# andywag/streaming_data_loader

Measured on AMD Instinct MI355X. Metric: device-resident tokenize+mask MB/s of input text, seq_len=512, 1/2/4/8 MI355X, higher is better.
Workload: dtype u8->int32

## Files before the change

streaming_data_loader_amd/csrc/kernels.hpp:

```cpp
#pragma once

#include <hip/hip_runtime.h>

#include <cstdint>

#include "common.hpp"
#include "zstd_format.hpp"

namespace sdl {

hipError_t launch_chunk_ranges(const uint64_t *off, int64_t R, int64_t N, uint32_t *ranges, hipStream_t st,
                               uint32_t *rb1 = nullptr, uint32_t *zero1 = nullptr, const void *copy_src = nullptr,
                               void *copy_dst = nullptr, size_t copy_bytes = 0);

hipError_t launch_wordpiece_chunks(const DevTok &T, const DevFirst &F, bool cased, const uint8_t *text, int64_t N,
                                   const uint64_t *off, int64_t R,
                                   uint32_t *ranges, uint16_t *tokc, uint32_t *chunk_cnt, uint32_t *rec_local,
                                   hipStream_t st, int64_t c_begin = 0, int64_t c_end = -1);

struct BpeLong {
    uint64_t pos;
    uint32_t len;
    uint32_t chunk;
    uint32_t k;
// ... 110 lines not shown
                             uint64_t n_order, uint8_t *windows, uint16_t *gmaps, uint8_t *gwin, hipStream_t st);
hipError_t launch_gz_resolve(const uint16_t *slots, uint32_t cap, const uint32_t *order, const uint32_t *len,
                             const uint64_t *pos, uint64_t n_order, const uint8_t *windows, uint8_t *out,
                             uint32_t *crc, uint32_t *shift, const X2N &x2n, int32_t *status, hipStream_t st);
hipError_t launch_gz_crc_fold(const uint32_t *crc, const uint32_t *shift, uint64_t n_order, const uint8_t *trailer,
                              const int32_t *status, int32_t *mstatus, hipStream_t st);

int64_t scan_tmp_words(int64_t n);
hipError_t launch_exclusive_scan(const uint32_t *in, uint32_t *out, int64_t n, uint32_t *tmp, hipStream_t st,
                                 const uint32_t *carry_in = nullptr);
int64_t scan_small_max();

enum : int32_t {
    ZS_OK = zs::OK,
    ZS_E_RANGE = zs::E_RANGE,
    ZS_E_TRUNC = zs::E_TRUNC,
    ZS_E_MAGIC = zs::E_MAGIC,
    ZS_E_DICT = zs::E_DICT,
    ZS_E_WINDOW = zs::E_WINDOW,
    ZS_E_BTYPE = zs::E_BTYPE,
    ZS_E_BSIZE = zs::E_BSIZE,
    ZS_E_LITHDR = zs::E_LITHDR,
    ZS_E_HUF = zs::E_HUF,
    ZS_E_FSE = zs::E_FSE,
    ZS_E_SEQHDR = zs::E_SEQHDR,
    ZS_E_ENDBITS = zs::E_ENDBITS,
    ZS_E_FAR = zs::E_FAR,
    ZS_E_SIZE = zs::E_SIZE,
    ZS_E_CHECKSUM = zs::E_CHECKSUM,
    ZS_E_STALL = zs::E_STALL
};
hipError_t launch_zs_index(const uint8_t *zst, uint64_t len, const uint64_t *foff, uint64_t n, zs::Frame *frames,
                           zs::Block *blocks, const uint32_t *first_block, uint32_t *nblk, uint32_t block_cap,
                           hipStream_t st);
hipError_t launch_zs_parse(const uint8_t *zst, const zs::Frame *frames, zs::Block *blocks, uint32_t nb, hipStream_t st);
hipError_t launch_zs_link(zs::Frame *frames, zs::Block *blocks, uint64_t n, uint32_t *lit_tot, uint32_t *seq_tot,
                          unsigned long long *totals, hipStream_t st);
hipError_t launch_zs_decode(const uint8_t *zst, const zs::Frame *frames, zs::Block *blocks, uint32_t nb,
                            const uint32_t *lit_base, const uint32_t *seq_base, uint8_t *lit, zs::SeqRec *seq,
                            hipStream_t st);
hipError_t launch_zs_chain(zs::Frame *frames, zs::Block *blocks, uint64_t n, uint32_t *out_size,
                           unsigned long long *totals, hipStream_t st);
hipError_t launch_zs_write(const uint8_t *zst, zs::Frame *frames, const zs::Block *blocks, uint32_t nb, uint64_t n,
                           const uint32_t *lit_base, const uint32_t *seq_base, const uint8_t *lit, const zs::SeqRec *seq,
                           const uint32_t *ooff, uint8_t *out, bool check, int32_t *status, uint32_t *bad,
                           hipStream_t st, hipEvent_t *ev = nullptr);

constexpr int MAX_SEGMENTS = 16;
struct SegChunks {
    int64_t cb[MAX_SEGMENTS + 1];
    int K;
};
hipError_t launch_seg_bounds(const uint32_t *ranges, const SegChunks &sc, int64_t R, uint32_t *rb, hipStream_t st);
hipError_t launch_scan_range(const uint32_t *in, uint32_t *out, const uint32_t *rb, int k, hipStream_t st);

hipError_t launch_compact_tokens(const uint32_t *tokc, const uint32_t *chunk_cnt, const uint32_t *chunk_off,
                                 int64_t n_chunks, uint32_t *tok, const uint32_t *long_count,
                                 const uint32_t *chunk_ent, const BpeLong *long_list, const uint16_t *long_scratch,
                                 hipStream_t st, const uint32_t *long_pool = nullptr, int64_t stride = STAGE,
                                 bool list16 = false);


struct SegSel {
    const uint32_t *rb;
    int k;
    int last;
};

int64_t records_tile_words(int64_t R);
hipError_t launch_records(const RowParams &P, const uint64_t *off, int64_t R, int64_t N, const uint32_t *chunk_off,
                          int64_t n_chunks, const uint32_t *rec_local, uint32_t *rec_tok, uint32_t *rec_cnt,
                          uint32_t *rec_rows, SegSel sel, hipStream_t st, uint32_t *tile_sums = nullptr);

struct DirectDst {
    int32_t *ids[2], *am[2], *tt[2], *lab[2];
    uint32_t base, cap, B, pad;
};
struct RowOut {
    int32_t *input_ids, *attention_mask, *token_type_ids, *labels;
    float *labels_f32;
    DirectDst direct;
};

constexpr int64_t SMALL_CHUNKS = 64;
struct SmallDown {
    const uint32_t *tokc, *chunk_cnt;
    uint32_t *chunk_off, *tok;
    const uint32_t *long_count, *chunk_ent;
    const BpeLong *long_list;
    const uint16_t *long_scratch;
    const uint32_t *long_pool;
    int64_t stride;
    int list16;
    const uint32_t *rec_local;
    uint32_t *rec_tok, *rec_cnt, *rec_rows, *row_off, *row_rec;
    uint32_t *stat;
    const uint32_t *tok_err;
    int rows;
    RowOut out;
};
hipError_t launch_downstream_small(const SmallDown &d, const RowParams &P, const uint64_t *off, int64_t R, int64_t N,
                                   hipStream_t st);

struct TokSrc {
    const uint32_t *tok;
    const uint16_t *lists;
    const uint32_t *chunk_off;
    int64_t n_lists;
    const uint32_t *row_chunk;
};

struct RowChunkIn {
    uint32_t *row_chunk;
    const uint32_t *rec_tok, *rec_cnt, *chunk_off;
    const uint64_t *off;
    int64_t n_lists;
    int32_t S, n_pre, chunk;
};
hipError_t launch_row_map(const uint32_t *row_off, int64_t R, uint32_t *row_rec, SegSel sel, hipStream_t st,
                          const RowChunkIn *rc = nullptr);
hipError_t launch_scan_rows_map(const uint32_t *rec_rows, int64_t R, const uint32_t *tile_sums, uint32_t *row_off,
                                uint32_t *row_rec, hipStream_t st, const RowChunkIn *rc = nullptr);

struct RowSeg {
    int32_t *ids, *am, *tt, *lab;
    uint32_t g0, n, dst, pad;
};
hipError_t launch_rows_to_host(const RowSeg *segs, int n_segs, uint32_t rows_per_seg_max, const int32_t *ids,
                               const int32_t *am, const int32_t *tt, const int32_t *lab, int S, int LW,
                               hipStream_t st);

hipError_t launch_rows_direct(const DirectDst &d, const uint32_t *row_off, int64_t R, const int32_t *ids,
                              const int32_t *am, const int32_t *tt, const int32_t *lab, int S, int LW,
                              const uint32_t *err0, const uint32_t *err1, uint32_t *stat, hipStream_t st);

struct MaskPolicy {
    int32_t policy;
    int32_t per_mille;
    uint32_t vocab_size;
    uint32_t pad;
    const uint32_t *cont_bits;
};

hipError_t launch_rows(const RowParams &P, const TokSrc &src, const uint32_t *rec_tok, const uint32_t *rec_cnt,
                       const uint32_t *row_off, const uint32_t *row_rec, SegSel sel, int64_t rows_cap, RowOut out,
                       hipStream_t st,
                       hipStream_t st_late = nullptr, const MaskPolicy *mp = nullptr);
struct PackParams {
    const uint32_t *tok, *rec_tok, *rec_cnt;
    uint32_t *rec_len;
    uint32_t *pk_off;
    int64_t R, rows_cap;
    int32_t S, B, eos, min_ids;
    const int32_t *carry_ids, *carry_pos;
    const uint32_t *carry_len;
    int32_t *new_ids, *new_pos;
    uint32_t *new_len;
    int32_t *ids, *am, *lab, *pos;
    uint32_t *d_rows;
};
hipError_t launch_pack_lengths(const PackParams &q, hipStream_t st);
hipError_t launch_pack_rows(const PackParams &q, hipStream_t st);
hipError_t launch_pack_flush(const PackParams &q, hipStream_t st);

struct PairParams {
    const uint16_t *lists;
    const uint32_t *chunk_off;
    const uint64_t *off;
    int64_t n_lists;
    const uint32_t *rec_tok, *rec_cnt;
    int64_t n_pairs;
    int64_t rows_end;
    int32_t S, cls, sep, pad;
    int32_t *ids, *am, *tt;
    uint32_t *row_off, *row_rec, *rb;
};
hipError_t launch_rows_pair(const PairParams &q, hipStream_t st);

hipError_t launch_mask_rand_rec(const RowParams &P, uint32_t *list, uint32_t *spos, uint16_t *jbuf, uint32_t *bits,
                                hipStream_t st);
hipError_t launch_multi_labels(const uint32_t *labels, const uint64_t *label_off, const uint32_t *row_rec,
                               const uint32_t *row_off, SegSel sel, int64_t rows_cap, int B, int NL, float *out,
                               uint32_t *err, hipStream_t st);

struct SpanPlan {
    uint2 *tab;
    uint2 *meta;
    int32_t capr;
    uint32_t *ovf_list, *ovf_n;
};
hipError_t launch_rows_span(const RowParams &P, const uint32_t *tok, const uint32_t *rec_tok, const uint32_t *rec_cnt,
                            const uint32_t *row_off, const uint32_t *row_rec, SegSel sel, int64_t rows_cap,
                            RowOut out, uint32_t *err, hipStream_t st, const SpanPlan *plan = nullptr);

// ... 41 lines not shown
```

streaming_data_loader_amd/csrc/pipeline.hip:

```cpp
#include "common.hpp"
#include "device_util.hpp"
#include "kernels.hpp"
#include "rows_device.hpp"
#include "span_noise.hpp"

namespace sdl {

constexpr int SCAN_NT = 256;
constexpr int SCAN_PER = 8;
constexpr int SCAN_TILE = SCAN_NT * SCAN_PER;
constexpr int64_t SCAN_MAX_BLOCKS = 1024;

__global__ __launch_bounds__(SCAN_NT) void k_scan_reduce(const uint32_t *__restrict__ in, int64_t n,
                                                         uint32_t *__restrict__ sums, int64_t nb,
                                                         const uint32_t *carry_in) {
    __shared__ uint32_t scratch[SCAN_NT / 64];
    const int64_t base = (int64_t)blockIdx.x * SCAN_TILE + (int64_t)threadIdx.x * SCAN_PER;
    uint32_t s = 0;
#pragma unroll
    for (int k = 0; k < SCAN_PER; ++k)
        if (base + k < n) s += in[base + k];
    uint32_t tot;
    block_excl_sum<SCAN_NT>(s, &tot, scratch);
    if (threadIdx.x == 0) {
// ... 478 lines not shown
    ChaRow cr;
    chacha_row_init(cr, key);
    uint32_t *gnx = nx + (S + 1) * grp, *gbt = bt + bw * grp;
    for (int x = gl; x <= S; x += 16) gnx[x] = NONE;
    for (int x = gl; x < bw; x += 16) gbt[x] = 0u;
    int i = active ? S - 1 : 0;
    uint32_t n = (uint32_t)i + 1u, zone = (n << __builtin_clz(n)) - 1u;
    for (uint32_t blk = 0;; blk += 16) {
        const int irow = __builtin_amdgcn_update_dpp(0, i, 0x150, 0xF, 0xF, false);
        if (!__any(irow >= i0)) break;
        uint32_t o[16];
        chacha12_block_row(cr, blk + (uint32_t)gl, o);
        static_for<0, 16>([&](auto bc) {
            constexpr int b = decltype(bc)::value;
#pragma unroll
            for (int q = 0; q < 16; ++q) {
                const uint32_t x = (uint32_t)__builtin_amdgcn_update_dpp(0, (int)o[q], 0x150 + b, 0xF, 0xF, false);
                const uint64_t m = (uint64_t)x * n;
                const bool acc = i >= i0 && (uint32_t)m <= zone;
                const uint32_t j = (uint32_t)(m >> 32);
                if (gl == 0) atomicMin(&gnx[acc && j != (uint32_t)i ? j : (uint32_t)S], (uint32_t)i);
                i -= acc ? 1 : 0;
                n = (uint32_t)i + 1u;
                zone = (n << __builtin_clz(n)) - 1u;
            }
        });
    }
    wave_sync();
    if (active)
        for (int x = gl; x < kmask; x += 16) {
            uint32_t p = (uint32_t)x;
            for (uint32_t q = gnx[p]; q != NONE; q = gnx[p]) p = q;
            atomicOr(&gbt[p >> 5], 1u << (p & 31));
        }
    wave_sync();
}

template <int MR, bool RM1, bool LATE = false, bool LISTS = false>
__global__ __launch_bounds__(256) __attribute__((amdgpu_waves_per_eu(MR >= 4 ? ROWS_WAVES4 : LATE ? 4 : RM1 ? ROWS_WAVES_RM1 : ROWS_WAVES, 8))) void k_rows(RowParams P, TokSrc tok,
                                              const uint32_t *__restrict__ rec_tok, const uint32_t *__restrict__ rec_cnt,
                                              const uint32_t *__restrict__ row_off, const uint32_t *__restrict__ row_rec,
                                              SegSel sel, int64_t rows_cap, RowOut out) {
    const int lane = lane_id();
    const int wid = LISTS ? __builtin_amdgcn_readfirstlane((int)(threadIdx.x >> 6)) : (int)(threadIdx.x >> 6);
    constexpr int NXS = 256 * MR + 1, BW = 8 * MR;
    __shared__ __attribute__((aligned(16))) uint32_t s_rw[LATE ? 4 : 1][LATE ? 4 * (NXS + BW) : 1];
    const RowSpan rs = row_span(sel, row_off, P.B, rows_cap);
    const int64_t G = rs.g_real;
    const DirectDst &dd = out.direct;
    const int64_t g_end = dd.cap ? rs.g_real : rs.g_end;
    if constexpr (LATE) {
        for (int64_t g0 = rs.g_lo + ((int64_t)blockIdx.x * 4 + wid) * 64; g0 < G; g0 += (int64_t)gridDim.x * 256) {
            const int64_t gl = g0 + lane;
            bool late = false;
            if (gl < G) {
                const int64_t r = row_rec[gl];
                late = rand_pre_slot(P, r, (uint32_t)(gl - row_off[r])) < 0;
            }
            uint32_t *const rw = s_rw[LATE ? wid : 0];
            uint32_t *const bits = rw + 4 * NXS;
            for (uint64_t m = __ballot(late); m;) {
                const int nr = __popcll(m) < 4 ? __popcll(m) : 4;
                uint64_t mm = m;
                for (int q = 0; q < (lane >> 4) && mm; ++q) mm &= mm - 1;
                const int64_t gq = g0 + (mm ? __builtin_ctzll(mm) : 0);
                uint64_t rec = 0;
                uint32_t kq = 0;
                if ((lane >> 4) < nr) {
                    const int64_t r = row_rec[gq];
                    rec = P.first_record + (uint64_t)r;
                    kq = (uint32_t)(gq - row_off[r]);
                }
                rand_rows16(P, nr, rec, kq, rw, bits, BW, lane);
                for (int q = 0; q < nr; ++q, m &= m - 1)
                    row_one<MR, RM1, LATE, LISTS>(P, tok, rec_tok, rec_cnt, row_off, row_rec, g0 + __builtin_ctzll(m), G, out,
                                           bits + BW * q, lane);
                __builtin_amdgcn_wave_barrier();
            }
        }
    } else {
        for (int64_t g = rs.g_lo + (int64_t)blockIdx.x * 4 + wid; g < g_end; g += (int64_t)gridDim.x * 4)
            row_one<MR, RM1, LATE, LISTS>(P, tok, rec_tok, rec_cnt, row_off, row_rec, g, G, out, nullptr, lane);
    }
}

template <int MR, bool WHOLE, bool LISTS>
__global__ __launch_bounds__(256) void k_rows_policy(RowParams P, MaskPolicy mp, TokSrc tok,
                                                     const uint32_t *__restrict__ rec_tok,
                                                     const uint32_t *__restrict__ rec_cnt,
                                                     const uint32_t *__restrict__ row_off,
                                                     const uint32_t *__restrict__ row_rec, SegSel sel,
                                                     int64_t rows_cap, RowOut out) {
    const int lane = lane_id();
    const int wid = __builtin_amdgcn_readfirstlane((int)(threadIdx.x >> 6));
    __shared__ uint32_t s_unit[WHOLE ? 4 : 1][WHOLE ? 256 * MR : 1];
    const RowSpan rs = row_span(sel, row_off, P.B, rows_cap);
    const int64_t G = rs.g_real;
    const int64_t g_end = out.direct.cap ? rs.g_real : rs.g_end;
    for (int64_t g = rs.g_lo + (int64_t)blockIdx.x * 4 + wid; g < g_end; g += (int64_t)gridDim.x * 4)
        row_policy_one<MR, WHOLE, LISTS>(P, mp, tok, rec_tok, rec_cnt, row_off, row_rec, g, G, out,
                                         s_unit[WHOLE ? wid : 0], lane);
}

template <int MR>
__global__ __launch_bounds__(SCAN_SMALL_NT) void k_downstream_small(SmallDown d, RowParams P,
                                                                    const uint64_t *__restrict__ off, int64_t R,
                                                                    int64_t N, int64_t n_chunks) {
    __shared__ uint32_t scratch[SCAN_SMALL_NT / 64];
    block_scan_small(d.chunk_cnt, n_chunks, d.chunk_off, scratch);
    __syncthreads();
    for (int64_t cb = (int64_t)(threadIdx.x >> 6) * COMPACT_CPW; cb < n_chunks;
         cb += (int64_t)(SCAN_SMALL_NT / 64) * COMPACT_CPW)
        compact_small(d, cb, d.chunk_off, n_chunks);
    for (int64_t r = threadIdx.x; r < R; r += SCAN_SMALL_NT)
        record_one(P, off, r, N, d.chunk_off, n_chunks, d.rec_local, d.rec_tok, d.rec_cnt, d.rec_rows);
    __syncthreads();
    block_scan_small(d.rec_rows, R, d.row_off, scratch);
    __syncthreads();
    for (int64_t r = threadIdx.x; r < R; r += SCAN_SMALL_NT)
        for (uint32_t g = d.row_off[r]; g < d.row_off[r + 1]; ++g) d.row_rec[g] = (uint32_t)r;
    if (d.stat) {
        for (int64_t r = threadIdx.x; r <= R; r += SCAN_SMALL_NT) d.stat[r] = d.row_off[r];
        if (threadIdx.x == 0) {
            d.stat[R + 1] = 0u;
            d.stat[R + 2] = d.tok_err ? *d.tok_err : 0u;
        }
    }
    if constexpr (MR > 0) {
        __syncthreads();
        const int64_t G = (int64_t)d.row_off[R];
        const int64_t g_end = d.out.direct.cap ? G : (G + P.B - 1) / P.B * P.B;
        for (int64_t g = (int64_t)(threadIdx.x >> 6); g < g_end; g += SCAN_SMALL_NT / 64)
            row_one<MR, false, false>(P, TokSrc{d.tok}, d.rec_tok, d.rec_cnt, d.row_off, d.row_rec, g, G, d.out, nullptr,
                                      lane_id());
    }
}

template <int MR>
__global__ __launch_bounds__(64) void k_downstream_tiny(SmallDown d, RowParams P, const uint64_t *__restrict__ off,
                                                        int64_t R, int64_t N, int64_t n_chunks) {
    downstream_tiny<MR>(d, P, off, R, N, n_chunks);
}

hipError_t launch_downstream_small(const SmallDown &d, const RowParams &P, const uint64_t *off, int64_t R, int64_t N,
                                   hipStream_t st) {
    const int64_t n_chunks = (N + CHUNK - 1) / CHUNK;
    if (n_chunks > SMALL_CHUNKS || R > SCAN_SMALL) return hipErrorInvalidValue;
    const int MR = (P.S + 255) / 256;
    if (d.rows && ((P.rng_mode == 1 && P.task == 0) || (P.task != 0 && P.task != 1)))
        return hipErrorInvalidValue;
    const bool tiny = R <= 64 && n_chunks <= 64;
#define LAUNCH_DS(M)                                                                                                    \
    if (tiny) hipLaunchKernelGGL(k_downstream_tiny<M>, dim3(1), dim3(64), 0, st, d, P, off, R, N, n_chunks);        \
    else hipLaunchKernelGGL(k_downstream_small<M>, dim3(1), dim3(SCAN_SMALL_NT), 0, st, d, P, off, R, N, n_chunks)
    if (!d.rows) LAUNCH_DS(0);
    else if (MR <= 1) LAUNCH_DS(1);
    else if (MR <= 2) LAUNCH_DS(2);
    else if (MR <= 4) LAUNCH_DS(4);
    else if (MR <= 8) LAUNCH_DS(8);
    else return hipErrorInvalidValue;
#undef LAUNCH_DS
    return hipGetLastError();
}

template <int NR>
__device__ __forceinline__ void rand_walk_lanes(const RowParams &P, const bool (&active)[NR], const uint64_t (&rec)[NR],
// ... 237 lines not shown
                                                     int S, int LW, const uint32_t *__restrict__ err0,
                                                     const uint32_t *__restrict__ err1, uint32_t *__restrict__ stat) {
    if (blockIdx.x == 0) {
        for (int64_t r = threadIdx.x; r <= R; r += 256) stat[r] = row_off[r];
        if (threadIdx.x == 0) {
            stat[R + 1] = err0 ? *err0 : 0u;
            stat[R + 2] = err1 ? *err1 : 0u;
        }
    }
    const uint32_t total = row_off[R];
    const uint32_t n = total < d.cap ? total : d.cap;
    const int plane = (int)(threadIdx.x >> 6), lane = (int)(threadIdx.x & 63);
    const int32_t *src = plane == 0 ? ids : plane == 1 ? am : plane == 2 ? tt : lab;
    if (!src) return;
    const int W = plane == 3 ? LW : S;
    const bool vec = (W & 3) == 0;
    for (uint32_t g = blockIdx.x; g < n; g += gridDim.x) {
        const uint32_t slot = d.base + g, bi = slot >= d.B ? 1u : 0u, row = slot - bi * d.B;
        int32_t *dst = plane == 0 ? d.ids[bi] : plane == 1 ? d.am[bi] : plane == 2 ? d.tt[bi] : d.lab[bi];
        const int32_t *s = src + (size_t)g * W;
        int32_t *o = dst + (size_t)row * W;
        if (vec && ((uintptr_t)dst & 15u) == 0) {
            for (int j = 4 * lane; j < W; j += 256)
                *reinterpret_cast<int4 *>(o + j) = *reinterpret_cast<const int4 *>(s + j);
        } else {
            for (int j = lane; j < W; j += 64) o[j] = s[j];
        }
    }
}

hipError_t launch_rows_direct(const DirectDst &d, const uint32_t *row_off, int64_t R, const int32_t *ids,
                              const int32_t *am, const int32_t *tt, const int32_t *lab, int S, int LW,
                              const uint32_t *err0, const uint32_t *err1, uint32_t *stat, hipStream_t st) {
    const unsigned grid = d.cap < 64u ? (d.cap ? d.cap : 1u) : 64u;
    hipLaunchKernelGGL(k_rows_direct, dim3(grid), dim3(256), 0, st, d, row_off, R, ids, am, tt, lab, S, LW, err0, err1,
                       stat);
    return hipGetLastError();
}

hipError_t launch_rows(const RowParams &P, const TokSrc &tok, const uint32_t *rec_tok, const uint32_t *rec_cnt,
                       const uint32_t *row_off, const uint32_t *row_rec, SegSel sel, int64_t rows_cap, RowOut out,
                       hipStream_t st, hipStream_t st_late, const MaskPolicy *mp) {
    if (!st_late) st_late = st;
    if (rows_cap == 0) return hipSuccess;
    if (mp && mp->policy != 0) {
        if (P.task != 0 || P.rng_mode != 0 || mp->policy < 1 || mp->policy > 2 || P.label_width != P.S ||
            !out.labels || (mp->policy == 2 && !mp->cont_bits))
            return hipErrorInvalidValue;
        const int64_t want_p = (rows_cap + 3) / 4;
        const unsigned grid_p = (unsigned)(want_p < 16384 ? want_p : 16384);
        const int MRp = (P.S + 255) / 256;
#define LAUNCH_POLICY_L(MM, WW, LL)                                                                                     \
    hipLaunchKernelGGL((k_rows_policy<MM, WW, LL>), dim3(grid_p), dim3(256), 0, st, P, *mp, tok, rec_tok, rec_cnt,   \
                       row_off, row_rec, sel, rows_cap, out)
#define LAUNCH_POLICY(MM)                                                                                               \
    do {                                                                                                              \
        if (mp->policy == 2) {                                                                                        \
            if (tok.lists) LAUNCH_POLICY_L(MM, true, true);                                                           \
            else LAUNCH_POLICY_L(MM, true, false);                                                                    \
        } else {                                                                                                      \
            if (tok.lists) LAUNCH_POLICY_L(MM, false, true);                                                          \
            else LAUNCH_POLICY_L(MM, false, false);                                                                   \
        }                                                                                                             \
    } while (0)
        if (MRp <= 1) LAUNCH_POLICY(1);
        else if (MRp <= 2) LAUNCH_POLICY(2);
        else if (MRp <= 4) LAUNCH_POLICY(4);
        else if (MRp <= 8) LAUNCH_POLICY(8);
        else return hipErrorInvalidValue;
#undef LAUNCH_POLICY
#undef LAUNCH_POLICY_L
        return hipGetLastError();
    }
constexpr int ROWS_GRID_CAP = 16384;
    const int64_t want = (rows_cap + 3) / 4;
    const unsigned grid = (unsigned)(want < ROWS_GRID_CAP ? want : ROWS_GRID_CAP);
    const int MR = (P.S + 255) / 256;
    if (P.label_width > 256 * MR) return hipErrorInvalidValue;
    const bool rm1 = P.task == 0 && P.rng_mode == 1;
    if (rm1 && ((P.mask_bits0 && !P.mask_off) || P.mask_w * 32 < P.S || P.S > RAND_MAX_S))
        return hipErrorInvalidValue;
    const int64_t want_late = (rows_cap + 255) / 256;
    const unsigned grid_late = (unsigned)(want_late < 2048 ? want_late : 2048);
#define LAUNCH_ROWS_L(MM, LL)                                                                                           \
    if (rm1) {                                                                                                        \
        hipLaunchKernelGGL((k_rows<MM, true, false, LL>), dim3(grid), dim3(256), 0, st, P, tok, rec_tok, rec_cnt,    \
                           row_off, row_rec, sel, rows_cap, out);                                                     \
        hipLaunchKernelGGL((k_rows<MM, true, true, LL>), dim3(grid_late), dim3(256), 0, st_late, P, tok, rec_tok,    \
                           rec_cnt, row_off, row_rec, sel, rows_cap, out);                                            \
    } else                                                                                                            \
        hipLaunchKernelGGL((k_rows<MM, false, false, LL>), dim3(grid), dim3(256), 0, st, P, tok, rec_tok, rec_cnt,   \
                           row_off, row_rec, sel, rows_cap, out)
#define LAUNCH_ROWS(MM)                                                                                                 \
    do {                                                                                                              \
        if (tok.lists) {                                                                                              \
            LAUNCH_ROWS_L(MM, true);                                                                                  \
        } else {                                                                                                      \
            LAUNCH_ROWS_L(MM, false);                                                                                 \
        }                                                                                                             \
    } while (0)
    if (MR <= 1) LAUNCH_ROWS(1);
    else if (MR <= 2) LAUNCH_ROWS(2);
    else if (MR <= 4) LAUNCH_ROWS(4);
    else if (MR <= 8) LAUNCH_ROWS(8);
    else return hipErrorInvalidValue;
#undef LAUNCH_ROWS
#undef LAUNCH_ROWS_L
    return hipGetLastError();
}

__device__ __forceinline__ uint32_t span_pick(int32_t kmin, int32_t n, const uint32_t (&thr)[32], uint32_t x) {
    int32_t v = kmin;
#pragma unroll
    for (int j = 0; j < 32; ++j) v += (j < n && thr[j] <= x) ? 1 : 0;
    return (uint32_t)v;
}

constexpr int SPAN_WBLK = 17;
constexpr int SPAN_WU64 = 8 * SPAN_WBLK;
constexpr double ZIG_R = 3.6541528853610088;

struct SpanStream {
    uint32_t key[8];
    const uint32_t *win;
    uint64_t wblk;
    uint32_t cblk[16];
    int64_t chave;
    __device__ uint64_t at(uint64_t k) {
        const uint64_t b = k >> 3;
        uint32_t lo, hi;
        if (b - wblk < (uint64_t)SPAN_WBLK) {
            const uint32_t w = (uint32_t)(2 * (k - 8 * wblk));
            lo = win[w];
            hi = win[w + 1];
        } else {
            if ((int64_t)b != chave) {
                chacha12_block(key, (uint32_t)b, cblk);
                chave = (int64_t)b;
            }
            lo = cblk[2 * (k & 7)];
            hi = cblk[2 * (k & 7) + 1];
        }
        return (uint64_t)hi << 32 | lo;
    }
};

__device__ __forceinline__ double bits_f64(uint64_t b) { return __longlong_as_double((long long)b); }

__device__ __forceinline__ bool zig_fast(uint64_t bits, const double *__restrict__ ZX, double *x) {
#pragma clang fp contract(off)
    const int i = (int)(bits & 0xffu);
    const double u = bits_f64((bits >> 12) | (1024ull << 52)) - 3.0;
    *x = u * ZX[i];
    return fabs(*x) < ZX[i + 1];
}

template <class Stream>
__device__ double zig_normal(Stream &s, uint64_t k, const double *__restrict__ ZX,
                             const double *__restrict__ ZF, uint32_t *len) {
#pragma clang fp contract(off)
    const uint64_t k0 = k;
    for (;;) {
        const uint64_t bits = s.at(k++);
        const int i = (int)(bits & 0xffu);
        const double u = bits_f64((bits >> 12) | (1024ull << 52)) - 3.0;
        const double x = u * ZX[i];
// ... 868 lines not shown
```

streaming_data_loader_amd/csrc/rows_device.hpp:

```cpp
#pragma once
#include "common.hpp"
#include "device_util.hpp"
#include "kernels.hpp"
#include "list_index.hpp"
#include "mlm_pick.hpp"

namespace sdl {

static_assert(LIST_CHUNK == CHUNK && LIST_STRIDE == STAGE, "list_index.hpp restates the chunk geometry");

constexpr int COMPACT_CPW = 4;
template <int PART = 0, bool E16 = false>
__device__ __forceinline__ void compact_wave(int64_t cb, const uint32_t *__restrict__ tokc,
                                             const uint32_t *__restrict__ chunk_cnt,
                                             const uint32_t *__restrict__ chunk_off, int64_t n_chunks,
                                             uint32_t *__restrict__ tok, const uint32_t *long_count,
                                             const uint32_t *__restrict__ chunk_ent,
                                             const BpeLong *__restrict__ long_list,
                                             const uint16_t *__restrict__ long_scratch,
                                             const uint32_t *__restrict__ long_pool, int64_t stride) {
    const int lane = threadIdx.x & 63;
    uint32_t n[COMPACT_CPW], o[COMPACT_CPW];
#pragma unroll
    for (int j = 0; j < COMPACT_CPW; ++j) {
// ... 404 lines not shown
            mwd[m] = j0 < S && mine ? bw[j0 >> 5] : 0u;
        }
        if (LATE) __builtin_amdgcn_wave_barrier();
    }

    const RowIds<MR> ids = row_ids<MR, LISTS>(P, src, c, bnd, nl, t0, cnt, base, l, lane);
    const int32_t (&id)[MR][4] = ids.v;
    if (RM1 && !mine) return;
    const int tail0 = l < S ? S - l : S;
    const uint64_t rec = P.first_record + (uint64_t)r;
    if (P.task == 0) {
        bool sel[MR][4];
        if (RM1) {
#pragma unroll
            for (int m = 0; m < MR; ++m) {
                const int j0 = 256 * m + 4 * lane;
#pragma unroll
                for (int w = 0; w < 4; ++w) sel[m][w] = (mwd[m] >> ((j0 + w) & 31)) & 1u;
            }
        } else {
            uint32_t key[MR][4];
#pragma unroll
            for (int m = 0; m < MR; ++m) {
                const uint4 c = philox4x32_10(make_uint4((uint32_t)(64 * m + lane), k, (uint32_t)rec,
                                                         (uint32_t)(rec >> 32)),
                                              (uint32_t)P.seed, (uint32_t)(P.seed >> 32));
                const int j0 = 256 * m + 4 * lane;
                key[m][0] = j0 < S ? c.x : 0xFFFFFFFFu;
                key[m][1] = j0 + 1 < S ? c.y : 0xFFFFFFFFu;
                key[m][2] = j0 + 2 < S ? c.z : 0xFFFFFFFFu;
                key[m][3] = j0 + 3 < S ? c.w : 0xFFFFFFFFu;
            }
            select_k_smallest_interp<MR>(key, P.mask_length, S < 256 * MR ? S : 256 * MR, sel);
        }
#pragma unroll
        for (int m = 0; m < MR; ++m) {
            const int j0 = 256 * m + 4 * lane;
            int32_t v[4], lab[4], am[4];
#pragma unroll
            for (int w = 0; w < 4; ++w) {
                v[w] = id[m][w];
                lab[w] = -100;
                if (sel[m][w] && v[w] != 0) {
                    lab[w] = v[w];
                    v[w] = P.mask_id;
                }
                am[w] = j0 + w >= tail0 ? 0 : 1;
            }
            store4(ids_o, j0, S, vec, v[0], v[1], v[2], v[3]);
            store4(am_o, j0, S, vec, am[0], am[1], am[2], am[3]);
            if (tt_o) store4(tt_o, j0, S, vec, 0, 0, 0, 0);
            store4(lb_o, j0, P.label_width, vec_lb, lab[0], lab[1], lab[2], lab[3]);
        }
    } else if (P.task == 3 || P.task == 4) {
#pragma unroll
        for (int m = 0; m < MR; ++m) {
            const int j0 = 256 * m + 4 * lane;
            int32_t am[4];
#pragma unroll
            for (int w = 0; w < 4; ++w) am[w] = j0 + w >= tail0 ? 0 : 1;
            store4(ids_o, j0, S, vec, id[m][0], id[m][1], id[m][2], id[m][3]);
            store4(am_o, j0, S, vec, am[0], am[1], am[2], am[3]);
            if (tt_o) store4(tt_o, j0, S, vec, 0, 0, 0, 0);
        }
    } else {
#pragma unroll
        for (int m = 0; m < MR; ++m) {
            const int j0 = 256 * m + 4 * lane;
            int32_t am[4], lab[4];
#pragma unroll
            for (int w = 0; w < 4; ++w) {
                const bool tail = j0 + w >= tail0;
                am[w] = tail ? 0 : 1;
                lab[w] = tail ? -100 : id[m][w];
            }
            store4(ids_o, j0, S, vec, id[m][0], id[m][1], id[m][2], id[m][3]);
            store4(am_o, j0, S, vec, am[0], am[1], am[2], am[3]);
            if (tt_o) store4(tt_o, j0, S, vec, 0, 0, 0, 0);
            store4(lb_o, j0, P.label_width, vec_lb, lab[0], lab[1], lab[2], lab[3]);
        }
    }
}

__device__ __forceinline__ uint32_t max_u32(uint32_t a, uint32_t b) { return a > b ? a : b; }
__device__ __forceinline__ uint32_t min_u32r(uint32_t a, uint32_t b) { return a < b ? a : b; }
struct PickWave {
    uint32_t l;
    __device__ __forceinline__ uint32_t sum(uint32_t x) const {
        return (uint32_t)__builtin_amdgcn_readlane((int)wave_incl_sum(x), 63);
    }
    __device__ __forceinline__ uint32_t min(uint32_t x) const {
        DPP_SCAN_ID(x, min_u32r, 0xFFFFFFFFu);
        return (uint32_t)__builtin_amdgcn_readlane((int)x, 63);
    }
    __device__ __forceinline__ uint32_t lane() const { return l; }
};

template <int MR, bool WHOLE, bool LISTS>
__device__ __forceinline__ void row_policy_one(const RowParams &P, const MaskPolicy &mp, const TokSrc &src,
                                               const uint32_t *__restrict__ rec_tok,
                                               const uint32_t *__restrict__ rec_cnt,
                                               const uint32_t *__restrict__ row_off,
                                               const uint32_t *__restrict__ row_rec, int64_t g, int64_t G,
                                               const RowOut &out, uint32_t *lds, int lane) {
    const int S = P.S;
    const bool vec = (S & 3) == 0;
    const DirectDst &dd = out.direct;
    int32_t *ids_o = out.input_ids + g * S;
    int32_t *am_o = out.attention_mask + g * S;
    int32_t *tt_o = out.token_type_ids ? out.token_type_ids + g * S : nullptr;
    int32_t *lb_o = out.labels + g * (int64_t)S;
    if (g < (int64_t)dd.cap) {
        const uint32_t slot = dd.base + (uint32_t)g, bi = slot >= dd.B ? 1u : 0u, row = slot - bi * dd.B;
        ids_o = dd.ids[bi] + (size_t)row * S;
        am_o = dd.am[bi] + (size_t)row * S;
        tt_o = dd.tt[bi] ? dd.tt[bi] + (size_t)row * S : nullptr;
        lb_o = dd.lab[bi] + (size_t)row * S;
    }
    if (g >= (int64_t)G) {
#pragma unroll
        for (int m = 0; m < MR; ++m) {
            const int j0 = 256 * m + 4 * lane;
            store4(ids_o, j0, S, vec, 0, 0, 0, 0);
            store4(am_o, j0, S, vec, 1, 1, 1, 1);
            if (tt_o) store4(tt_o, j0, S, vec, 0, 0, 0, 0);
            store4(lb_o, j0, S, vec, -100, -100, -100, -100);
        }
        return;
    }
    const int64_t nl = LISTS ? src.n_lists : 0;
    uint32_t c = 0, bnd = 0;
    if constexpr (LISTS) {
        c = (uint32_t)__builtin_amdgcn_readfirstlane((int)src.row_chunk[g]);
        bnd = src.chunk_off[(int64_t)c + lane < nl ? (int64_t)c + lane : nl];
    }
    const int64_t r = row_rec[g];
    const uint32_t ck = (uint32_t)(g - row_off[r]);
    const uint32_t cnt = rec_cnt[r];
    const uint32_t t0 = rec_tok[r];
    const int64_t n = (int64_t)cnt + P.n_pre + P.n_post;
    const int64_t base = P.chunk ? (int64_t)ck * S : 0;
    const int l = (int)((n - base) < S ? (n - base) : S);
    const RowIds<MR> ids = row_ids<MR, LISTS>(P, src, c, bnd, nl, t0, cnt, base, l, lane);
    const int32_t (&id)[MR][4] = ids.v;
    const int tail0 = l < S ? S - l : S;
    const uint64_t rec = P.first_record + (uint64_t)r;
    const PickWave wv{(uint32_t)lane};

    uint32_t cand = 0;
#pragma unroll
    for (int m = 0; m < MR; ++m)
#pragma unroll
        for (int w = 0; w < 4; ++w) {
            const int32_t v = id[m][w];
            bool ex = v == 0 || v == P.mask_id;
#pragma unroll
            for (int q = 0; q < MAX_FRAME; ++q)
                ex = ex || (q < P.n_pre && v == frame_id(P.pre, q)) || (q < P.n_post && v == frame_id(P.post, q));
            if (256 * m + 4 * lane + w < l && !ex) cand |= 1u << (4 * m + w);
        }
    const int ncand = (int)wv.sum((uint32_t)__popc(cand));
    int kb = (int)(((int64_t)l * mp.per_mille + 500) / 1000);
    kb = kb < 1 ? 1 : kb;
    kb = kb < P.mask_length ? kb : P.mask_length;
    if (ncand == 0) kb = 0;

// ... 183 lines not shown
```

Baseline: 241,500.

## Add specialized fast row-building kernel reading args from kernarg segment

Adds a k_rows_fast kernel, specialised per task, for the common row-building configuration: aligned S, no direct destinations, default RNG mode. It reads parameters straight from the kernarg segment with scalar-pinned reloads to keep register pressure down, sets waves-per-EU occupancy hints, and writes output with vectorised nontemporal stores. The aim is to cut VGPR/SGPR pressure and branching in the generic row kernel, at the cost of a second code path that has to stay semantically in sync with the original (padding rows, frames, MLM selection).

```diff
diff --git a/streaming_data_loader_amd/csrc/kernels.hpp b/streaming_data_loader_amd/csrc/kernels.hpp
--- a/streaming_data_loader_amd/csrc/kernels.hpp
+++ b/streaming_data_loader_amd/csrc/kernels.hpp
@@ -216,6 +216,13 @@
     DirectDst direct;
 };
 
+struct RowFast {
+    int32_t *input_ids, *attention_mask, *token_type_ids, *labels;
+    uint64_t seed, first_record;
+    int32_t S, B, chunk, mask_length, mask_id, n_pre, n_post, pad;
+    int32_t pre[MAX_FRAME], post[MAX_FRAME];
+};
+
 constexpr int64_t SMALL_CHUNKS = 64;
 struct SmallDown {
     const uint32_t *tokc, *chunk_cnt;
@@ -244,6 +251,15 @@
     const uint32_t *row_chunk;
 };
 
+struct RowsFastArgs {
+    RowFast F;
+    TokSrc tok;
+    const uint32_t *rec_tok, *rec_cnt, *row_off, *row_rec;
+    const uint32_t *rb;
+    int32_t k, last;
+    int64_t rows_cap;
+};
+
 struct RowChunkIn {
     uint32_t *row_chunk;
     const uint32_t *rec_tok, *rec_cnt, *chunk_off;
diff --git a/streaming_data_loader_amd/csrc/pipeline.hip b/streaming_data_loader_amd/csrc/pipeline.hip
--- a/streaming_data_loader_amd/csrc/pipeline.hip
+++ b/streaming_data_loader_amd/csrc/pipeline.hip
@@ -584,6 +584,24 @@
         for (int64_t g = rs.g_lo + (int64_t)blockIdx.x * 4 + wid; g < g_end; g += (int64_t)gridDim.x * 4)
             row_one<MR, RM1, LATE, LISTS>(P, tok, rec_tok, rec_cnt, row_off, row_rec, g, G, out, nullptr, lane);
     }
+}
+
+template <int MR, int TASK, bool LISTS>
+__global__ __launch_bounds__(256) __attribute__((amdgpu_waves_per_eu(MR >= 4 ? ROWS_WAVES4 : ROWS_WAVES, 8))) void k_rows_fast(
+    RowsFastArgs A) {
+    const int lane = lane_id();
+    const uint32_t wid = (uint32_t)__builtin_amdgcn_readfirstlane((int)(threadIdx.x >> 6));
+    const uint32_t g_lo = A.row_off[A.rb[A.k]], G = A.row_off[A.rb[A.k + 1]], step = gridDim.x * 4u;
+    uint32_t g_end = G;
+    if (A.last) {
+        const uint32_t B = (uint32_t)A.F.B, cap = (uint32_t)A.rows_cap;
+        uint32_t pad = (G + B - 1u) / B * B;
+        pad = pad > cap ? cap : pad;
+        g_end = pad > G ? pad : G;
+    }
+    const RowArgs a = (RowArgs)__builtin_amdgcn_kernarg_segment_ptr();
+    for (uint32_t g = g_lo + blockIdx.x * 4u + wid; g < g_end; g += step)
+        row_fast_one<MR, TASK, LISTS>(a, g, G, lane);
 }
 
 template <int MR, bool WHOLE, bool LISTS>
@@ -987,6 +1005,41 @@
         return hipErrorInvalidValue;
     const int64_t want_late = (rows_cap + 255) / 256;
     const unsigned grid_late = (unsigned)(want_late < 2048 ? want_late : 2048);
+    const bool label_task = P.task == 3 || P.task == 4;
+    const bool fast = (P.S & 3) == 0 && out.direct.cap == 0 && P.rng_mode == 0 && rows_cap < (int64_t(1) << 31) &&
+                      (label_task || ((P.task == 0 || P.task == 1) && out.labels && P.label_width == P.S));
+    if (fast) {
+        RowsFastArgs A{RowFast{out.input_ids, out.attention_mask, out.token_type_ids, label_task ? nullptr : out.labels,
+                               P.seed, P.first_record, P.S, P.B, P.chunk, P.mask_length, P.mask_id, P.n_pre, P.n_post,
+                               0, {}, {}},
+                       tok, rec_tok, rec_cnt, row_off, row_rec, sel.rb, sel.k, sel.last, rows_cap};
+        for (int q = 0; q < MAX_FRAME; ++q) {
+            A.F.pre[q] = P.pre[q];
+            A.F.post[q] = P.post[q];
+        }
+#define LAUNCH_FAST_L(MM, TT, LL)                                                                                       \
+    hipLaunchKernelGGL((k_rows_fast<MM, TT, LL>), dim3(grid), dim3(256), 0, st, A)
+#define LAUNCH_FAST(MM)                                                                                                 \
+    do {                                                                                                              \
+        if (tok.lists) {                                                                                              \
+            if (label_task) LAUNCH_FAST_L(MM, ROW_LABELS, true);                                                      \
+            else if (P.task == 0) LAUNCH_FAST_L(MM, ROW_MLM, true);                                                   \
+            else LAUNCH_FAST_L(MM, ROW_CLM, true);                                                                    \
+        } else {                                                                                                      \
+            if (label_task) LAUNCH_FAST_L(MM, ROW_LABELS, false);                                                     \
+            else if (P.task == 0) LAUNCH_FAST_L(MM, ROW_MLM, false);                                                  \
+            else LAUNCH_FAST_L(MM, ROW_CLM, false);                                                                   \
+        }                                                                                                             \
+    } while (0)
+        if (MR <= 1) LAUNCH_FAST(1);
+        else if (MR <= 2) LAUNCH_FAST(2);
+        else if (MR <= 4) LAUNCH_FAST(4);
+        else if (MR <= 8) LAUNCH_FAST(8);
+        else return hipErrorInvalidValue;
+#undef LAUNCH_FAST
+#undef LAUNCH_FAST_L
+        return hipGetLastError();
+    }
 #define LAUNCH_ROWS_L(MM, LL)                                                                                           \
     if (rm1) {                                                                                                        \
         hipLaunchKernelGGL((k_rows<MM, true, false, LL>), dim3(grid), dim3(256), 0, st, P, tok, rec_tok, rec_cnt,    \
diff --git a/streaming_data_loader_amd/csrc/rows_device.hpp b/streaming_data_loader_amd/csrc/rows_device.hpp
--- a/streaming_data_loader_amd/csrc/rows_device.hpp
+++ b/streaming_data_loader_amd/csrc/rows_device.hpp
@@ -510,6 +510,235 @@
     }
 }
 
+constexpr int ROW_MLM = 0, ROW_CLM = 1, ROW_LABELS = 2;
+
+typedef const __attribute__((address_space(4))) RowsFastArgs *RowArgs;
+__device__ __forceinline__ RowArgs row_args_again(RowArgs a) {
+    asm volatile("" : "+s"(a));
+    return a;
+}
+
+__device__ __forceinline__ void store4v(int32_t *p, int j0, int32_t a, int32_t b, int32_t c, int32_t d) {
+    typedef int32_t v4i __attribute__((ext_vector_type(4)));
+    __builtin_nontemporal_store(v4i{a, b, c, d}, reinterpret_cast<v4i *>(p + j0));
+}
+
+template <int MR, bool LISTS>
+__device__ __forceinline__ RowIds<MR> row_ids_fast(RowArgs a, uint32_t c, uint32_t bnd, int64_t nl, uint32_t t0,
+                                                   uint32_t cnt, int64_t base, int l, int lane) {
+    const int n_pre = a->F.n_pre;
+    const int64_t rel0 = base > n_pre ? base - n_pre : 0;
+    const int64_t rel1 = base + l - n_pre < (int64_t)cnt ? base + l - n_pre : (int64_t)cnt;
+    const int jlo = (int)(rel0 + n_pre - base), jhi = (int)(rel1 + n_pre - base);
+    const uint32_t tb = t0 + (uint32_t)(base - n_pre);
+    RowIds<MR> out;
+#pragma unroll
+    for (int m = 0; m < MR; ++m)
+#pragma unroll
+        for (int w = 0; w < 4; ++w) out.v[m][w] = 0;
+    if (rel0 < rel1) {
+        uint32_t t[MR][4];
+#pragma unroll
+        for (int m = 0; m < MR; ++m)
+#pragma unroll
+            for (int w = 0; w < 4; ++w) {
+                const int j = 256 * m + 4 * lane + w;
+                const int jc = j < jlo ? jlo : j > jhi - 1 ? jhi - 1 : j;
+                t[m][w] = tb + (uint32_t)jc;
+            }
+        if constexpr (LISTS) {
+            const uint32_t t_last = (uint32_t)__builtin_amdgcn_readfirstlane((int)(tb + (uint32_t)(jhi - 1)));
+            const uint16_t *__restrict__ lc = a->tok.lists + (int64_t)c * STAGE;
+            if ((uint32_t)__builtin_amdgcn_readlane((int)bnd, 63) > t_last) {
+                uint32_t q[MR][4];
+#pragma unroll
+                for (int m = 0; m < MR; ++m)
+#pragma unroll
+                    for (int w = 0; w < 4; ++w) q[m][w] = 0;
+#pragma unroll 1
+                for (int b = 1; b < 64; ++b) {
+                    const uint32_t x = (uint32_t)__builtin_amdgcn_readlane((int)bnd, b);
+                    if (x > t_last) break;
+#pragma unroll
+                    for (int m = 0; m < MR; ++m)
+#pragma unroll
+                        for (int w = 0; w < 4; ++w) q[m][w] += t[m][w] >= x ? 1u : 0u;
+                }
+#pragma unroll
+                for (int m = 0; m < MR; ++m)
+#pragma unroll
+                    for (int w = 0; w < 4; ++w) {
+                        const uint32_t lo = (uint32_t)__shfl((int)bnd, (int)(q[m][w] & 63u));
+                        out.v[m][w] = (int32_t)lc[q[m][w] * (uint32_t)STAGE + (t[m][w] - lo)];
+                    }
+            } else {
+                const uint32_t *const chunk_off = a->tok.chunk_off;
+                const uint16_t *const lists = a->tok.lists;
+#pragma unroll 1
+                for (int i = 0; i < 4 * MR; ++i) {
+                    uint32_t ti = 0;
+#pragma unroll
+                    for (int m = 0; m < MR; ++m)
+#pragma unroll
+                        for (int w = 0; w < 4; ++w) ti = i == 4 * m + w ? t[m][w] : ti;
+                    const int64_t cc = list_chunk_of(chunk_off, (int64_t)c, nl - 1, ti);
+                    const int32_t v = (int32_t)lists[list_slot(chunk_off, cc, ti)];
+#pragma unroll
+                    for (int m = 0; m < MR; ++m)
+#pragma unroll
+                        for (int w = 0; w < 4; ++w) out.v[m][w] = i == 4 * m + w ? v : out.v[m][w];
+                }
+            }
+        } else {
+            const uint32_t *const tok = a->tok.tok;
+#pragma unroll
+            for (int m = 0; m < MR; ++m)
+#pragma unroll
+                for (int w = 0; w < 4; ++w) out.v[m][w] = (int32_t)tok[t[m][w]];
+        }
+    }
+    a = row_args_again(a);
+    static_assert(MAX_FRAME == 4, "the frame selects below");
+    int32_t p0 = a->F.pre[0], p1 = a->F.pre[1], p2 = a->F.pre[2], p3 = a->F.pre[3];
+    int32_t q0 = a->F.post[0], q1 = a->F.post[1], q2 = a->F.post[2], q3 = a->F.post[3];
+    asm volatile("" : "+s"(p0), "+s"(p1), "+s"(p2), "+s"(p3), "+s"(q0), "+s"(q1), "+s"(q2), "+s"(q3));
+    auto frame4 = [](int k, int32_t x0, int32_t x1, int32_t x2, int32_t x3) {
+        int32_t x = x3;
+        x = k == 2 ? x2 : x;
+        x = k == 1 ? x1 : x;
+        x = k == 0 ? x0 : x;
+        return x;
+    };
+    const int post0 = (int)(base - n_pre - (int64_t)cnt);
+#pragma unroll
+    for (int m = 0; m < MR; ++m)
+#pragma unroll
+        for (int w = 0; w < 4; ++w) {
+            const int j = 256 * m + 4 * lane + w;
+            int32_t v = out.v[m][w];
+            if (m == 0) {
+                const int32_t f = frame4((int)base + j, p0, p1, p2, p3);
+                v = j < jlo ? f : v;
+            }
+            const int32_t f = frame4(post0 + j, q0, q1, q2, q3);
+            v = j >= jhi ? f : v;
+            out.v[m][w] = j < l ? v : 0;
+        }
+    return out;
+}
+
+template <int MR>
+struct RowIn {
+    bool r[MR];
+};
+template <int MR>
+__device__ __forceinline__ RowIn<MR> row_in(int S, int lane) {
+    RowIn<MR> x;
+#pragma unroll
+    for (int m = 0; m < MR; ++m) x.r[m] = m < MR / 2 || 256 * m + 4 * lane < S;
+    return x;
+}
+
+template <int MR, int TASK>
+__device__ __forceinline__ void row_fast_store(RowArgs a, uint32_t g, int lane, const int32_t (&v)[MR][4],
+                                               const int32_t (&am)[MR][4], const int32_t (&lab)[MR][4]) {
+    a = row_args_again(a);
+    const int S = a->F.S;
+    const RowIn<MR> in = row_in<MR>(S, lane);
+    const int64_t o = (int64_t)g * S;
+    int32_t *const ids_o = a->F.input_ids + o, *const am_o = a->F.attention_mask + o;
+    int32_t *const lb_o = TASK != ROW_LABELS ? a->F.labels + o : nullptr;
+    int32_t *const tt = a->F.token_type_ids;
+#pragma unroll
+    for (int m = 0; m < MR; ++m)
+        if (in.r[m]) {
+            const int j0 = 256 * m + 4 * lane;
+            store4v(ids_o, j0, v[m][0], v[m][1], v[m][2], v[m][3]);
+            store4v(am_o, j0, am[m][0], am[m][1], am[m][2], am[m][3]);
+            if constexpr (TASK != ROW_LABELS) store4v(lb_o, j0, lab[m][0], lab[m][1], lab[m][2], lab[m][3]);
+        }
+    if (tt) {
+#pragma unroll
+        for (int m = 0; m < MR; ++m)
+            if (in.r[m]) store4v(tt + o, 256 * m + 4 * lane, 0, 0, 0, 0);
+    }
+}
+
+template <int MR, int TASK, bool LISTS>
+__device__ __forceinline__ void row_fast_one(RowArgs a, uint32_t g, uint32_t G, int lane) {
+    int32_t v[MR][4], am[MR][4], lab[MR][4];
+    if (g >= G) {
+#pragma unroll
+        for (int m = 0; m < MR; ++m)
+#pragma unroll
+            for (int w = 0; w < 4; ++w) {
+                v[m][w] = 0;
+                am[m][w] = 1;
+                lab[m][w] = -100;
+            }
+        row_fast_store<MR, TASK>(a, g, lane, v, am, lab);
+        return;
+    }
+    a = row_args_again(a);
+    const int S = a->F.S;
+    const int64_t nl = LISTS ? a->tok.n_lists : 0;
+    uint32_t c = 0, bnd = 0;
+    if constexpr (LISTS) {
+        c = (uint32_t)__builtin_amdgcn_readfirstlane((int)a->tok.row_chunk[g]);
+        bnd = a->tok.chunk_off[(int64_t)c + lane < nl ? (int64_t)c + lane : nl];
+    }
+    const uint32_t r = a->row_rec[g];
+    const uint32_t k = g - a->row_off[r];
+    const uint32_t cnt = a->rec_cnt[r];
+    const uint32_t t0 = a->rec_tok[r];
+    const int64_t n = (int64_t)cnt + a->F.n_pre + a->F.n_post;
+    const int64_t base = a->F.chunk ? (int64_t)k * S : 0;
+    const int l = (int)((n - base) < S ? (n - base) : S);
+    const RowIds<MR> ids = row_ids_fast<MR, LISTS>(a, c, bnd, nl, t0, cnt, base, l, lane);
+    const int32_t (&id)[MR][4] = ids.v;
+    const int tail0 = l < S ? S - l : S;
+    if constexpr (TASK == ROW_MLM) {
+        a = row_args_again(a);
+        const uint64_t rec = a->F.first_record + (uint64_t)r;
+        const uint64_t seed = a->F.seed;
+        const RowIn<MR> in = row_in<MR>(S, lane);
+        uint32_t key[MR][4];
+        bool sel[MR][4];
+#pragma unroll
+        for (int m = 0; m < MR; ++m) {
+            const uint4 x = philox4x32_10(make_uint4((uint32_t)(64 * m + lane), k, (uint32_t)rec, (uint32_t)(rec >> 32)),
+                                          (uint32_t)seed, (uint32_t)(seed >> 32));
+            key[m][0] = in.r[m] ? x.x : 0xFFFFFFFFu;
+            key[m][1] = in.r[m] ? x.y : 0xFFFFFFFFu;
+            key[m][2] = in.r[m] ? x.z : 0xFFFFFFFFu;
+            key[m][3] = in.r[m] ? x.w : 0xFFFFFFFFu;
+        }
+        select_k_smallest_interp<MR>(key, a->F.mask_length, S, sel);
+        a = row_args_again(a);
+        const int32_t mask_id = a->F.mask_id;
+#pragma unroll
+        for (int m = 0; m < MR; ++m)
+#pragma unroll
+            for (int w = 0; w < 4; ++w) {
+                const bool pick = sel[m][w] && id[m][w] != 0;
+                v[m][w] = pick ? mask_id : id[m][w];
+                lab[m][w] = pick ? id[m][w] : -100;
+                am[m][w] = 256 * m + 4 * lane + w >= tail0 ? 0 : 1;
+            }
+    } else {
+#pragma unroll
+        for (int m = 0; m < MR; ++m)
+#pragma unroll
+            for (int w = 0; w < 4; ++w) {
+                const bool tail = 256 * m + 4 * lane + w >= tail0;
+                v[m][w] = id[m][w];
+                am[m][w] = tail ? 0 : 1;
+                lab[m][w] = tail ? -100 : id[m][w];
+            }
+    }
+    row_fast_store<MR, TASK>(a, g, lane, v, am, lab);
+}
+
 __device__ __forceinline__ uint32_t max_u32(uint32_t a, uint32_t b) { return a > b ? a : b; }
 __device__ __forceinline__ uint32_t min_u32r(uint32_t a, uint32_t b) { return a < b ? a : b; }
 struct PickWave {
```

Measured after the change: 250,500 (median of 6 runs). +3.7%, better.
